# UoB-HPC/stdpar-nbody

Measured on AMD Instinct MI355X. Metric: body-steps/sec + %FP64 peak, 3D double all-pairs N=2^20 at 1/2/4/8 GPUs, higher is better.
Workload: dtype f64

## Files before the change

### stdpar-nbody_amd/csrc/all_pairs.hip

```cpp
#include "common.hpp"

#include <atomic>
#include <cstdlib>
#include <mutex>
#include <type_traits>
#include <vector>

namespace nbody {

constexpr int kBlock = 256;
constexpr int kWaves = kBlock / 64;

struct ap_config {
  int split = 0;
  int tpt   = 0;
  int path  = 0;
};
static std::atomic<uint32_t> g_ap_default{0};

static ap_config ap_config_of(const nbody_state* s) {
  const uint32_t t = s->tuning ? s->tuning : g_ap_default.load(std::memory_order_relaxed);
  ap_config c;
  c.split = int(t & 15u);
  c.tpt   = int((t >> 4) & 3u);
// ... 2 lines not shown
}

template <typename T, int D, int R, int JS>
__global__ __launch_bounds__(kBlock) void all_pairs_force_kernel(const T* __restrict__ m, const T* __restrict__ x,
                                                                 T* __restrict__ a, T c, uint32_t sz, uint32_t first,
                                                                 uint32_t count, const k1_rule* __restrict__ rule) {
  [[maybe_unused]] constexpr T e2 = T(0);
#define K1_SOFT false
#include "k1_tile_body.inc"
#undef K1_SOFT
}
template <typename T, int D, int R, int JS>
__global__ __launch_bounds__(kBlock) void all_pairs_softened_kernel(const T* __restrict__ m, const T* __restrict__ x,
                                                                    T* __restrict__ a, T c, uint32_t sz, uint32_t first,
                                                                    uint32_t count, T e2) {
  const k1_rule* const rule = nullptr;
#define K1_SOFT true
#include "k1_tile_body.inc"
#undef K1_SOFT
}

template <typename T, int D>
__global__ __launch_bounds__(kBlock) void pack_sources_kernel(const T* __restrict__ m, const T* __restrict__ x,
                                                              src_rec<T, D>* __restrict__ out, uint32_t sz, uint32_t padded) {
  const uint32_t j = blockIdx.x * kBlock + threadIdx.x;
  if (j >= padded) return;
  src_rec<T, D> r;
#pragma unroll
  for (int k = 0; k < 3; ++k) r.p[k] = (k < D && j < sz) ? x[uint64_t(j) * D + (k < D ? k : 0)] : T(0);
  r.m    = j < sz ? m[j] : T(0);
  out[j] = r;
}

template <typename T, int D, bool PACK, bool MOMENTS>
__global__ __launch_bounds__(kBlock) void k1_prepare_kernel(const T* __restrict__ m, const T* __restrict__ x, src_rec<T, D>* __restrict__ out,
                                                            cst_batch* __restrict__ cst, uint32_t sz, uint32_t padded, k1_rule* rule, double* partial,
                                                            uint32_t* turn, uint32_t turn_words) {
  const uint32_t j = blockIdx.x * kBlock + threadIdx.x;
  T p[D];
#pragma unroll
  for (int k = 0; k < D; ++k) p[k] = j < sz ? x[uint64_t(j) * D + k] : T(0);
  if constexpr (PACK) {
    if (j < padded) {
      src_rec<T, D> r;
#pragma unroll
      for (int k = 0; k < 3; ++k) r.p[k] = k < D ? p[k < D ? k : 0] : T(0);
      r.m    = j < sz ? m[j] : T(0);
      out[j] = r;
      if constexpr (sizeof(T) == 8) {
        const src_cst<T> k  = src_cst<T>::of(r.m);
        cst[j / 2].m15[j % 2]   = k.m15;
        cst[j / 2].m1875[j % 2] = k.m1875;
      }
    }
  }
  __shared__ double red[2 * D][kWaves];
  __shared__ bool last_s;
  const int lane = threadIdx.x & 63, wave = threadIdx.x >> 6;
  if constexpr (MOMENTS) {
    double s1[D], s2[D];
#pragma unroll
    for (int k = 0; k < D; ++k) {
      const double d = j < sz ? double(p[k]) - double(x[k]) : 0.0;
      s1[k] = d;
      s2[k] = d * d;
    }
#pragma unroll
    for (int k = 0; k < D; ++k)
      for (int off = 32; off > 0; off >>= 1) {
        s1[k] += __shfl_xor(s1[k], off, 64);
        s2[k] += __shfl_xor(s2[k], off, 64);
      }
    if (lane == 0) {
#pragma unroll
      for (int k = 0; k < D; ++k) {
        red[k][wave]     = s1[k];
        red[D + k][wave] = s2[k];
      }
    }
    __syncthreads();
    if (threadIdx.x < 2 * D) {
      double v = red[threadIdx.x][0];
      for (int w = 1; w < kWaves; ++w) v += red[threadIdx.x][w];
      __hip_atomic_store(partial + size_t(blockIdx.x) * (2 * D) + threadIdx.x, v, __ATOMIC_RELAXED, __HIP_MEMORY_SCOPE_AGENT);
    }
  }
  __builtin_amdgcn_s_waitcnt(0);
  __syncthreads();
  if (threadIdx.x == 0) last_s = __hip_atomic_fetch_add(&rule->ticket, 1u, __ATOMIC_RELAXED, __HIP_MEMORY_SCOPE_AGENT) == gridDim.x - 1u;
  __syncthreads();
  if (!last_s) return;
  if constexpr (MOMENTS) {
    double acc = 0.0;
    constexpr int G = kBlock / (2 * D), U = 8;
    const int q = threadIdx.x % (2 * D), g = threadIdx.x / (2 * D);
    if (g < G) {
      for (uint32_t b0 = uint32_t(g); b0 < gridDim.x; b0 += G * U) {
        double v[U];
#pragma unroll
        for (int u = 0; u < U; ++u) {
          const uint32_t b = b0 + uint32_t(u) * G;
          v[u] = b < gridDim.x ? __hip_atomic_load(partial + size_t(b) * (2 * D) + q, __ATOMIC_RELAXED, __HIP_MEMORY_SCOPE_AGENT) : 0.0;
        }
#pragma unroll
        for (int u = 0; u < U; ++u) acc += v[u];
      }
    }
    __shared__ double fin[kBlock];
    fin[threadIdx.x] = g < G ? acc : 0.0;
    __syncthreads();
    if (threadIdx.x < 2 * D) {
      double tot = 0.0;
#pragma unroll 6
      for (int gg = 0; gg < G; ++gg) tot += fin[gg * (2 * D) + threadIdx.x];
      fin[threadIdx.x] = tot;
    }
    __syncthreads();
    if (threadIdx.x == 0) {
      double vol = 1.0;
#pragma unroll
      for (int k = 0; k < D; ++k) {
        const double mean = fin[k] / double(sz), var = fin[D + k] / double(sz) - mean * mean;
        vol *= var > 0.0 ? __builtin_sqrt(12.0 * var) : 0.0;
      }
      rule->volume = vol;
      rule->sparse = vol >= kFarMinVolume<D> ? 1u : 0u;
    }
  }
  for (uint32_t w = threadIdx.x; w < turn_words; w += kBlock) turn[w] = 0u;
  if (threadIdx.x == 0) __hip_atomic_store(&rule->ticket, 0u, __ATOMIC_RELAXED, __HIP_MEMORY_SCOPE_AGENT);
}

template <int JS>
constexpr int kSgprWaves = JS > kWaves ? JS : kWaves;

constexpr uint32_t kTurnSpins  = 1u << 26;
constexpr uint32_t kTurnPoison = 0xffffffffu;
struct k1_status {
  uint32_t err, block, group, chunk;
  unsigned long long polls, waits;
};
struct k1_handoff {
  void* sums;
  uint32_t* turn;
  k1_status* status;
  uint32_t spins;
  uint32_t delay;
  uint32_t late;
};
template <typename T, int D, int R, int JS, int RULE = 0>
__global__ __launch_bounds__(64 * kSgprWaves<JS>) void all_pairs_force_sgpr_kernel(const src_rec<T, D>* __restrict__ packed,
                                                                                   const cst_batch* __restrict__ cst,
                                                                                   const T* __restrict__ x, T* a, T c, uint32_t sz,
                                                                                   uint32_t first, uint32_t count,
                                                                                   uint32_t tiles_per_chunk, k1_handoff h,
                                                                                   const k1_rule* __restrict__ rule) {
  [[maybe_unused]] constexpr T e2 = T(0);
#define K1_SOFT false
#include "k1_sgpr_body.inc"
#undef K1_SOFT
}
template <typename T, int D, int R, int JS>
__global__ __launch_bounds__(64 * kSgprWaves<JS>) void all_pairs_softened_sgpr_kernel(const src_rec<T, D>* __restrict__ packed,
                                                                                      const cst_batch* __restrict__ cst,
                                                                                      const T* __restrict__ x, T* a, T c, uint32_t sz,
                                                                                      uint32_t first, uint32_t count,
                                                                                      uint32_t tiles_per_chunk, k1_handoff h, T e2) {
  constexpr int RULE = 0;
  const k1_rule* const rule = nullptr;
#define K1_SOFT true
#include "k1_sgpr_body.inc"
#undef K1_SOFT
}

namespace {
struct scratch_buf {
  void* ptr  = nullptr;
  size_t cap = 0;
};
struct packed_slot {
  int device;
  hipStream_t stream;
  scratch_buf buf[7];
  std::vector<void*> retired;
  bool k1_dirty  = false;
  bool k1_failed = false;
};
std::mutex g_packed_mu;
std::vector<packed_slot> g_packed_slots;
}

int ap_scratch_get(hipStream_t st, int which, size_t bytes, void** out) {
  const int dev = stream_device(st);
  std::lock_guard<std::mutex> lock(g_packed_mu);
  packed_slot* slot = nullptr;
  for (auto& sl : g_packed_slots)
    if (sl.stream == st && sl.device == dev) slot = &sl;
  if (slot && slot->buf[which].cap >= bytes) {
    *out = slot->buf[which].ptr;
    return NBODY_OK;
  }
  hipStreamCaptureStatus cs = hipStreamCaptureStatusNone;
  if (st != nullptr) (void)hipStreamIsCapturing(st, &cs);
  if (cs != hipStreamCaptureStatusNone) {
    set_error("all-pairs: the scratch buffers of this stream must exist before a step is recorded "
              "(call nbody_all_pairs_force once outside nbody_graph_begin/end, or use a context from nbody_create)");
    return NBODY_ERR_STATE;
  }
  if (!slot) {
    g_packed_slots.push_back({dev, st, {}, {}});
    slot = &g_packed_slots.back();
  }
  void* fresh = nullptr;
  NB_HIP(hipMalloc(&fresh, bytes));
  if (which == 4 || which == 3) {
    if (hipError_t e = hipMemsetAsync(fresh, 0, bytes, st); e != hipSuccess) {
      (void)hipFree(fresh);
      return hip_fail(e, "hipMemsetAsync(K1 scratch)", __FILE__, __LINE__);
    }
  }
  if (slot->buf[which].ptr) slot->retired.push_back(slot->buf[which].ptr);
  slot->buf[which].ptr = fresh;
  slot->buf[which].cap = bytes;
  *out                 = fresh;
  return NBODY_OK;
}

void ap_scratch_release(hipStream_t st) {
  const int dev = stream_device(st);
  std::lock_guard<std::mutex> lock(g_packed_mu);
  for (size_t i = 0; i < g_packed_slots.size(); ++i) {
    if (g_packed_slots[i].stream == st && g_packed_slots[i].device == dev) {
      for (auto& b : g_packed_slots[i].buf) (void)hipFree(b.ptr);
      for (void* p : g_packed_slots[i].retired) (void)hipFree(p);
      g_packed_slots.erase(g_packed_slots.begin() + long(i));
      return;
    }
  }
}

struct k1_plan {
  bool scalar = false;
  int r = 1, js = 4;
  uint32_t chunks = 1, tiles_per_chunk = 0;
};

static int auto_split(uint32_t sz) { return sz >= 2048u ? 8 : 4; }

// ... 33 lines not shown
  if (p.r == 0) {
    const uint64_t blocks_r2 = (uint64_t(s->count) + 127) / 128 * p.chunks;
    if (p.scalar) p.r = (sizeof(T) == 8 && blocks_r2 >= 4096) ? 2 : 1;
    else p.r = blocks_r2 * uint64_t(p.js) >= 8192 ? 2 : 1;
  }
  *out = p;
  return NBODY_OK;
}

int ap_pack_sources(const nbody_state* s, hipStream_t st, void** packed_out) {
  const uint32_t padded = (s->sz + kTileJ - 1) / kTileJ * kTileJ;
  const size_t tsz      = s->dtype == NBODY_F32 ? 4 : 8;
  void* scratch         = nullptr;
  if (int r = ap_scratch_get(st, 0, 4 * tsz * size_t(padded), &scratch)) return r;
  int rc = dispatch(s->dtype, s->dim, [&](auto tg) {
    using T         = typename decltype(tg)::type;
    constexpr int D = decltype(tg)::dim;
    hipLaunchKernelGGL((pack_sources_kernel<T, D>), dim3((padded + kBlock - 1) / kBlock), dim3(kBlock), 0, st,
                       static_cast<const T*>(s->m), static_cast<const T*>(s->x), static_cast<src_rec<T, D>*>(scratch), s->sz, padded);
    NB_HIP(hipGetLastError());
    return int(NBODY_OK);
  });
  *packed_out = scratch;
  return rc;
}

static size_t ap_cst_bytes(size_t padded) { return sizeof(cst_batch) * (padded / 2); }

static size_t ap_rule_bytes(uint32_t sz, int dim) {
  const size_t padded = (size_t(sz) + kTileJ - 1) / kTileJ * kTileJ;
  return 32 + sizeof(double) * 2 * size_t(dim) * (padded / kBlock);
}

template <typename T, int D>
static int ap_prepare(const nbody_state* s, hipStream_t st, bool pack, src_rec<T, D>** packed_out, const cst_batch** cst_out,
                      const k1_rule** rule_out, uint32_t* turn, size_t turn_words, bool with_rule = true) {
  const uint32_t padded = (s->sz + kTileJ - 1) / kTileJ * kTileJ;
  const bool moments    = with_rule && s->sz >= kFarMinBodies;
  void* scratch         = nullptr;
  void* consts          = nullptr;
  if (pack) {
    if (int r = ap_scratch_get(st, 0, 4 * sizeof(T) * size_t(padded), &scratch)) return r;
    if (sizeof(T) == 8)
      if (int r = ap_scratch_get(st, 6, ap_cst_bytes(padded), &consts)) return r;
  }
  void* q = nullptr;
  if (int r = ap_scratch_get(st, 3, ap_rule_bytes(s->sz, D), &q)) return r;
  auto* rule    = static_cast<k1_rule*>(q);
  auto* partial = reinterpret_cast<double*>(static_cast<char*>(q) + 32);
  auto* out     = static_cast<src_rec<T, D>*>(scratch);
  auto* cst     = static_cast<cst_batch*>(consts);
  const dim3 grid(padded / kBlock), block(kBlock);
  const T *m = static_cast<const T*>(s->m), *x = static_cast<const T*>(s->x);
  const uint32_t words = uint32_t(turn_words);
  if (pack && moments) hipLaunchKernelGGL((k1_prepare_kernel<T, D, true, true>), grid, block, 0, st, m, x, out, cst, s->sz, padded, rule, partial, turn, words);
  else if (pack) hipLaunchKernelGGL((k1_prepare_kernel<T, D, true, false>), grid, block, 0, st, m, x, out, cst, s->sz, padded, rule, partial, turn, words);
  else if (moments) hipLaunchKernelGGL((k1_prepare_kernel<T, D, false, true>), grid, block, 0, st, m, x, out, cst, s->sz, padded, rule, partial, turn, words);
  NB_HIP(hipGetLastError());
  if (packed_out) *packed_out = out;
  if (cst_out) *cst_out = cst;
  *rule_out = moments ? rule : nullptr;
  return NBODY_OK;
}

constexpr uint32_t kCollectMaxBlocks = 2048;
static bool k1_collect(uint32_t target_blocks, uint32_t chunks) {
  uint32_t limit = kCollectMaxBlocks;
  if (const char* e = experiment_env("NBODY_K1_COLLECT_MAX")) limit = uint32_t(atoi(e));
  return chunks > 1 && uint64_t(target_blocks) * chunks <= limit;
}
template <typename T, int D, int R, int JS>
static size_t k1_collect_bytes(uint32_t target_blocks, uint32_t chunks) {
  constexpr int TG = kSgprWaves<JS> / JS;
  return sizeof(T) * size_t(chunks) * target_blocks * TG * R * D * 64;
}

template <int R, int JS>
static size_t sgpr_turn_words(uint32_t count) {
  constexpr int TG = kSgprWaves<JS> / JS, TB = TG * 64 * R;
  return size_t((count + TB - 1) / TB) * TG;
}

template <typename T, int D, int R, int JS, bool SOFT>
static int launch_all_pairs_sgpr(const nbody_state* s, const k1_plan& plan, hipStream_t st, T e2) {
  constexpr int TB = (kSgprWaves<JS> / JS) * 64 * R;
  uint32_t blocks  = (s->count + TB - 1) / TB;
  if (blocks == 0) return NBODY_OK;
  k1_handoff h{nullptr, nullptr, nullptr, kTurnSpins, 0u, 0u};
  if (plan.chunks > 1) {
    void* q = nullptr;
    if (int r = ap_scratch_get(st, 1, sizeof(uint32_t) * sgpr_turn_words<R, JS>(s->count), &q)) return r;
    h.turn = static_cast<uint32_t*>(q);
    if (k1_collect(blocks, plan.chunks)) {
      if (int r = ap_scratch_get(st, 5, k1_collect_bytes<T, D, R, JS>(blocks, plan.chunks), &q)) return r;
      h.sums = q;
    }
    if (int r = ap_scratch_get(st, 4, sizeof(k1_status), &q)) return r;
    h.status = static_cast<k1_status*>(q);
    if (const char* e = experiment_env("NBODY_K1_TURN_SPINS")) h.spins = uint32_t(strtoul(e, nullptr, 10));
    if (const char* e = experiment_env("NBODY_K1_HANDOFF_DELAY")) h.delay = uint32_t(strtoul(e, nullptr, 10));
    if (const char* e = experiment_env("NBODY_K1_HANDOFF_LATE")) h.late = uint32_t(strtoul(e, nullptr, 10));
    if (const char* e = experiment_env("NBODY_K1_NO_HANDOFF"); e && e[0] == '1') h.turn = nullptr, h.sums = nullptr;
    if (const char* e = experiment_env("NBODY_K1_COLLECT"); e && e[0] == '0') h.sums = nullptr;
  }
  src_rec<T, D>* packed = nullptr;
  const cst_batch* cst  = nullptr;
  const k1_rule* rule   = nullptr;
  if (int r = ap_prepare<T, D>(s, st, true, &packed, &cst, &rule, h.turn, h.turn ? sgpr_turn_words<R, JS>(s->count) : 0, !SOFT)) return r;
  if constexpr (SOFT) {
    hipLaunchKernelGGL((all_pairs_softened_sgpr_kernel<T, D, R, JS>), dim3(blocks, plan.chunks), dim3(64 * kSgprWaves<JS>), 0, st,
                       packed, cst, static_cast<const T*>(s->x), static_cast<T*>(s->a), static_cast<T>(s->c), s->sz, s->first, s->count,
                       plan.tiles_per_chunk, h, e2);
    NB_HIP(hipGetLastError());
    if (h.turn != nullptr && h.sums == nullptr) ap_status_mark(st);
    return NBODY_OK;
  }
#ifdef NBODY_EXPERIMENTS
  if (const char* e = getenv("NBODY_K1_RULE_FORCE"); e && JS == 8 && D == 3) {
    if (e[0] == '1')
      hipLaunchKernelGGL((all_pairs_force_sgpr_kernel<T, D, R, JS, 1>), dim3(blocks, plan.chunks), dim3(64 * kSgprWaves<JS>), 0, st,
                         packed, cst, static_cast<const T*>(s->x), static_cast<T*>(s->a), static_cast<T>(s->c), s->sz, s->first, s->count,
                         plan.tiles_per_chunk, h, rule);
    else
      hipLaunchKernelGGL((all_pairs_force_sgpr_kernel<T, D, R, JS, 2>), dim3(blocks, plan.chunks), dim3(64 * kSgprWaves<JS>), 0, st,
                         packed, cst, static_cast<const T*>(s->x), static_cast<T*>(s->a), static_cast<T>(s->c), s->sz, s->first, s->count,
                         plan.tiles_per_chunk, h, rule);
    NB_HIP(hipGetLastError());
    return NBODY_OK;
  }
#endif
  hipLaunchKernelGGL((all_pairs_force_sgpr_kernel<T, D, R, JS>), dim3(blocks, plan.chunks), dim3(64 * kSgprWaves<JS>), 0, st,
                     packed, cst, static_cast<const T*>(s->x), static_cast<T*>(s->a), static_cast<T>(s->c), s->sz, s->first, s->count,
                     plan.tiles_per_chunk, h, rule);
  NB_HIP(hipGetLastError());
  if (h.turn != nullptr && h.sums == nullptr) ap_status_mark(st);
  return NBODY_OK;
}

template <typename T, int D, int R, int JS, bool SOFT>
static int launch_all_pairs(const nbody_state* s, hipStream_t st, T e2) {
  constexpr int TB = (kWaves / JS) * 64 * R;
  uint32_t blocks  = (s->count + TB - 1) / TB;
  if (blocks == 0) return NBODY_OK;
  if constexpr (SOFT) {
    hipLaunchKernelGGL((all_pairs_softened_kernel<T, D, R, JS>), dim3(blocks), dim3(kBlock), 0, st, static_cast<const T*>(s->m),
                       static_cast<const T*>(s->x), static_cast<T*>(s->a), static_cast<T>(s->c), s->sz, s->first, s->count, e2);
    NB_HIP(hipGetLastError());
    return NBODY_OK;
  }
  const k1_rule* rule = nullptr;
  if (int r = ap_prepare<T, D>(s, st, false, nullptr, nullptr, &rule, nullptr, 0)) return r;
  hipLaunchKernelGGL((all_pairs_force_kernel<T, D, R, JS>), dim3(blocks), dim3(kBlock), 0, st, static_cast<const T*>(s->m),
                     static_cast<const T*>(s->x), static_cast<T*>(s->a), static_cast<T>(s->c), s->sz, s->first, s->count, rule);
  NB_HIP(hipGetLastError());
  return NBODY_OK;
}

template <typename F>
static bool with_k1_instance(const k1_plan& p, F&& fn) {
#define NB_CASE(RR, JJ)                                                                       \
  if (p.r == RR && p.js == JJ) {                                                              \
    fn(std::integral_constant<int, RR>{}, std::integral_constant<int, JJ>{});                 \
    return true;                                                                              \
  }
  NB_CASE(1, 1);
  NB_CASE(1, 2);
// ... 9 lines not shown
  return false;
}

template <typename T, int D, bool SOFT = false>
static int all_pairs_dispatch(const nbody_state* s, hipStream_t st, T e2 = T(0)) {
  k1_plan p;
  if (int rc = plan_all_pairs<T>(s, &p)) return rc;
  int rc = NBODY_OK;
  const bool found = with_k1_instance(p, [&](auto r, auto js) {
    constexpr int R = decltype(r)::value, JS = decltype(js)::value;
    rc = p.scalar ? launch_all_pairs_sgpr<T, D, R, JS, SOFT>(s, p, st, e2)
                  : (JS <= kWaves ? launch_all_pairs<T, D, R, (JS <= kWaves ? JS : 1), SOFT>(s, st, e2) : int(NBODY_ERR_ARG));
  });
  if (!found) {
    set_error("all-pairs: unsupported config split=%d targets_per_thread=%d", p.js, p.r);
    return NBODY_ERR_ARG;
  }
  return rc;
}

template <typename T, int D>
static int all_pairs_describe(const nbody_state* s, char* out, size_t len) {
  k1_plan p;
  if (int rc = plan_all_pairs<T>(s, &p)) return rc;
  const char* t = sizeof(T) == 8 ? "double" : "float";
  const char* pair = sizeof(T) == 4 ? (s->sz >= kFarMinBodies ? "rsq+rcp[m y^3 at r2 >= 4 if sparse]" : "rsq+rcp")
                                    : s->sz >= kFarMinBodies ? "far3m[-eps if sparse]/near3" : "far3m/near3";
  if (p.scalar) {
    bool collect = false;
    with_k1_instance(p, [&](auto r, auto js) {
      constexpr int TB = (kSgprWaves<decltype(js)::value> / decltype(js)::value) * 64 * decltype(r)::value;
      collect = k1_collect((s->count + TB - 1) / TB, p.chunks);
    });
    snprintf(out, len, "all_pairs_force_sgpr_kernel<%s,%d,R=%d,JS=%d> tile=%d chunks=%u%s pair=%s", t, D, p.r, p.js, kTileJ, p.chunks,
             p.chunks > 1 ? (collect ? "(summed in chunk order by the last to arrive)" : "(summed in turn into a)") : "", pair);
  }
  else
    snprintf(out, len, "all_pairs_force_kernel<%s,%d,R=%d,JS=%d> tile=%d chunks=1 pair=%s", t, D, p.r, p.js, kTileJ, pair);
  return NBODY_OK;
}

int ap_scratch_reserve(hipStream_t st, const nbody_state* s) {
  void* q             = nullptr;
  const size_t tsz    = s->dtype == NBODY_F32 ? 4 : 8;
  const size_t padded = (size_t(s->sz) + 2 * kTileJ - 1) / (2 * kTileJ) * (2 * kTileJ);
  if (int r = ap_scratch_get(st, 0, 4 * tsz * padded, &q)) return r;
  if (s->dtype == NBODY_F64)
    if (int r = ap_scratch_get(st, 6, ap_cst_bytes(padded), &q)) return r;
  if (int r = ap_scratch_get(st, 3, ap_rule_bytes(s->sz, s->dim), &q)) return r;
  return dispatch(s->dtype, s->dim, [&](auto tg) {
    using T = typename decltype(tg)::type;
    k1_plan p;
    if (int rc = plan_all_pairs<T>(s, &p)) return rc;
    if (!p.scalar || p.chunks <= 1) return int(NBODY_OK);
    size_t words = 0;
    with_k1_instance(p, [&](auto r, auto js) { words = sgpr_turn_words<decltype(r)::value, decltype(js)::value>(s->count); });
    if (!words) return int(NBODY_OK);
    if (int rc = ap_scratch_get(st, 1, sizeof(uint32_t) * words, &q)) return rc;
    size_t sums = 0;
    with_k1_instance(p, [&](auto r, auto js) {
      constexpr int RR = decltype(r)::value, JJ = decltype(js)::value;
      const uint32_t blocks = (s->count + (kSgprWaves<JJ> / JJ) * 64 * RR - 1) / ((kSgprWaves<JJ> / JJ) * 64 * RR);
      if (k1_collect(blocks, p.chunks)) sums = k1_collect_bytes<T, decltype(tg)::dim, RR, JJ>(blocks, p.chunks);
    });
    if (sums)
      if (int rc = ap_scratch_get(st, 5, sums, &q)) return rc;
    return ap_scratch_get(st, 4, sizeof(k1_status), &q);
  });
}

void ap_status_mark(hipStream_t st) {
  const int dev = stream_device(st);
  std::lock_guard<std::mutex> lock(g_packed_mu);
  for (auto& sl : g_packed_slots)
    if (sl.stream == st && sl.device == dev) sl.k1_dirty = true;
}

int ap_status_read(hipStream_t st, unsigned long long out[6], bool clear) {
  const int dev = stream_device(st);
  k1_status* dptr = nullptr;
  {
    std::lock_guard<std::mutex> lock(g_packed_mu);
// ... 610 lines not shown
  });
}

extern "C" int nbody_all_pairs_force(const nbody_state* s, void* stream) {
  if (int r = check_state(s)) return r;
  device_guard guard(stream_device(as_stream(stream)));
  return dispatch(s->dtype, s->dim, [&](auto tg) {
    using TG = decltype(tg);
    return all_pairs_dispatch<typename TG::type, TG::dim>(s, as_stream(stream));
  });
}

extern "C" int nbody_all_pairs_softened_force(const nbody_state* s, double eps, void* stream) {
  if (int r = check_state(s)) return r;
  return dispatch(s->dtype, s->dim, [&](auto tg) {
    using TG = decltype(tg);
    using T  = typename TG::type;
    T e2;
    if (int r = check_softening<T>(eps, &e2)) return r;
    device_guard guard(stream_device(as_stream(stream)));
    return all_pairs_dispatch<T, TG::dim, true>(s, as_stream(stream), e2);
  });
}

extern "C" int nbody_all_pairs_status(void* stream, uint64_t out[6], int clear) {
  device_guard guard(stream_device(as_stream(stream)));
  unsigned long long v[6] = {0, 0, 0, 0, 0, 0};
  const int rc = ap_status_read(as_stream(stream), v, clear != 0);
  if (out)
    for (int i = 0; i < 6; ++i) out[i] = v[i];
  return rc;
}

extern "C" int nbody_all_pairs_collapsed_force(const nbody_state* s, void* stream) {
  if (int r = check_state(s)) return r;
  device_guard guard(stream_device(as_stream(stream)));
  return dispatch(s->dtype, s->dim, [&](auto tg) {
    using TG = decltype(tg);
    return collapsed_dispatch<typename TG::type, TG::dim>(s, as_stream(stream));
  });
}

extern "C" int nbody_accelerate_step(const nbody_state* s, void* stream) {
  if (int r = check_state(s)) return r;
  device_guard guard(stream_device(as_stream(stream)));
  return dispatch(s->dtype, s->dim, [&](auto tg) {
    using TG = decltype(tg);
    return accelerate_dispatch<typename TG::type, TG::dim>(s, as_stream(stream));
  });
}
```

### stdpar-nbody_amd/csrc/common.hpp

```cpp
#pragma once
#include <hip/hip_runtime.h>

#include <cfloat>
#include <cstdarg>
#include <cstdint>
#include <cstdio>
#include <cstdlib>
#include <cstring>

#include "../../include/nbody_hip.h"

namespace nbody {

void set_error(const char* fmt, ...);
int hip_fail(hipError_t e, const char* what, const char* file, int line);

#define NB_HIP(call)                                                                   \
  do {                                                                                 \
    hipError_t e_ = (call);                                                            \
    if (e_ != hipSuccess) return ::nbody::hip_fail(e_, #call, __FILE__, __LINE__);     \
  } while (0)

#define NB_ARG(cond, ...)                \
  do {                                   \
// ... 343 lines not shown
#pragma unroll
      for (int u = 0; u < U; ++u)
#pragma unroll
        for (int r = 0; r < R; ++r) w[u][r] = pair_math<T>::template weight_far_folded<false>(r2[u][r], s[u].m, kc[u].m15, kc[u].m1875);
    } else {
#pragma unroll
      for (int u = 0; u < U; ++u)
#pragma unroll
        for (int r = 0; r < R; ++r) {
          const uint32_t hi = uint32_t(__builtin_bit_cast(unsigned long long, r2[u][r]) >> 32);
          const T mine      = hi < pair_math<T>::far_hi ? pc.keps : T(0);
          w[u][r]           = pair_math<T>::template weight_far_folded<true>(r2[u][r], s[u].m, kc[u].m15, kc[u].m1875, mine);
        }
      if (__builtin_expect(__builtin_amdgcn_ballot_w64(lowest < pair_math<T>::near_hi) != 0ull, 0)) {
#pragma unroll
        for (int u = 0; u < U; ++u)
#pragma unroll
          for (int r = 0; r < R; ++r) {
            const uint32_t hi = uint32_t(__builtin_bit_cast(unsigned long long, r2[u][r]) >> 32);
            const T wn        = pair_math<T>::template weight<3>(r2[u][r], s[u].m);
            w[u][r]           = hi < pair_math<T>::near_hi ? wn : w[u][r];
          }
      }
    }
#pragma unroll
    for (int u = 0; u < U; ++u)
#pragma unroll
      for (int r = 0; r < R; ++r)
#pragma unroll
        for (int k = 0; k < D; ++k) acc[r][k] = __builtin_elementwise_fma(w[u][r], d[u][r][k], acc[r][k]);
  }
}

template <typename T, int D, int R, int U, bool ffar>
__device__ __forceinline__ void pair_batch(T (&acc)[R][D], const T (&xi)[R][D], const src_rec<T, D> (&s)[U], const pair_consts<T>& pc) {
  static_assert(sizeof(T) == 4, "f64 callers pass the sources' constants (src_cst)");
  const src_cst<T> none[U] = {};
  pair_batch<T, D, R, U, ffar>(acc, xi, s, none, pc);
}

template <typename T>
__device__ __forceinline__ T soft_weight(T q, T mj, const pair_consts<T>& pc) {
  if constexpr (sizeof(T) == 8) {
    return pair_math<double>::template weight_far<false>(q, mj, pc.k15, pc.k1875);
  } else {
    const T y = __builtin_amdgcn_rsqf(q);
    return mj * ((y * y) * y);
  }
}

template <typename T, int D, int R, int U, bool SSRC = false>
__device__ __forceinline__ void pair_batch_soft(T (&acc)[R][D], const T (&xi)[R][D], const src_rec<T, D> (&s)[U],
                                                const src_cst<T> (&kc)[U], const pair_consts<T>& pc, T e2) {
  T d[U][R][D], q[U][R], w[U][R];
#pragma unroll
  for (int u = 0; u < U; ++u)
#pragma unroll
    for (int r = 0; r < R; ++r) {
#pragma unroll
      for (int k = 0; k < D; ++k) d[u][r][k] = s[u].p[k] - xi[r][k];
      T t = e2;
#pragma unroll
      for (int k = 0; k < D; ++k) t = __builtin_elementwise_fma(d[u][r][k], d[u][r][k], t);
      q[u][r] = t;
    }
#pragma unroll
// ... 12 lines not shown
      for (int k = 0; k < D; ++k) acc[r][k] = __builtin_elementwise_fma(w[u][r], d[u][r][k], acc[r][k]);
}

template <typename T>
constexpr T kSoftMinE2 = sizeof(T) == 4 ? T(0x1p-84f) : T(0x1p-680);

template <typename T>
inline int check_softening(double eps, T* e2_out) {
  NB_ARG(eps > 0.0 && eps <= DBL_MAX, "softening length eps = %g must be finite and > 0", eps);
  const T te = T(eps);
  const T e2 = te * te;
  NB_ARG(e2 >= kSoftMinE2<T> && e2 <= (sizeof(T) == 4 ? T(FLT_MAX) : T(DBL_MAX)),
         "softening length eps = %g: eps^2 = %g in %s is outside [%g, max]: its square must be a normal number whose ^(-3/2) is finite",
         eps, double(e2), sizeof(T) == 4 ? "float" : "double", double(kSoftMinE2<T>));
  *e2_out = e2;
  return NBODY_OK;
}

inline hipStream_t as_stream(void* s) { return reinterpret_cast<hipStream_t>(s); }

struct k1_rule {
  double volume;
  uint32_t sparse;
  uint32_t ticket;
};
constexpr uint32_t kFarMinBodies = 32768;
template <int D>
constexpr double kFarMinVolume = D == 3 ? 1.7e5 : 6.4e4;
__device__ __forceinline__ bool ap_far_mode(const k1_rule* __restrict__ rule) {
  if (rule == nullptr) return false;
  return __builtin_amdgcn_readfirstlane(int(rule->sparse)) != 0;
}

constexpr int kTileJ = 512;

typedef uint32_t sgpr16 __attribute__((ext_vector_type(16)));
template <typename V>
__device__ __forceinline__ sgpr16 sload16(const void* p, V& tie) {
  sgpr16 r;
  asm volatile("s_load_dwordx16 %0, %2, 0x0" : "=s"(r), "+v"(tie) : "s"(p));
  return r;
}
template <typename V>
__device__ __forceinline__ void swait(sgpr16& v, V& tie) {
  asm volatile("s_waitcnt lgkmcnt(0)" : "+s"(v), "+v"(tie));
}

typedef uint32_t reg4 __attribute__((ext_vector_type(4)));
struct cst_regs {
  reg4 v, s;
};
template <typename V>
__device__ __forceinline__ cst_regs cload(const void* p, uint32_t vzero, V& tie) {
  cst_regs r;
  asm volatile("global_load_dwordx4 %0, %3, %4\n\ts_load_dwordx4 %1, %4, 0x10" : "=&v"(r.v), "=&s"(r.s), "+v"(tie) : "v"(vzero), "s"(p));
  return r;
}
template <typename V>
__device__ __forceinline__ void cswait(sgpr16& v, cst_regs& c, V& tie) {
  asm volatile("s_waitcnt vmcnt(0) lgkmcnt(0)" : "+s"(v), "+v"(c.v), "+s"(c.s), "+v"(tie));
}
__device__ __forceinline__ void cst_unpack(const cst_regs& c, src_cst<double> (&kc)[2]) {
  struct pair_t {
    double d[2];
  };
  const pair_t v = __builtin_bit_cast(pair_t, c.v), s = __builtin_bit_cast(pair_t, c.s);
// ... 22 lines not shown
```

### stdpar-nbody_amd/csrc/k1_sgpr_body.inc

```
  using rec_t = src_rec<T, D>;
  constexpr int TG  = kSgprWaves<JS> / JS;
  constexpr int TB  = TG * 64 * R;
  constexpr int SUB = kTileJ / JS;
  __shared__ T partial[(JS > 1) ? (JS - 1) * TG * 64 * R * D : 1];
  const int lane   = threadIdx.x & 63;
  const int wave   = __builtin_amdgcn_readfirstlane(threadIdx.x >> 6);
  const int tgroup = wave / JS;
  const int jpart  = wave % JS;
  T xi[R][D], acc[R][D];
  uint32_t ti[R];
#pragma unroll
  for (int r = 0; r < R; ++r) {
    uint32_t local = blockIdx.x * TB + tgroup * (64 * R) + r * 64 + lane;
    ti[r]          = local;
    uint64_t i     = uint64_t(first) + (local < count ? local : 0u);
#pragma unroll
    for (int k = 0; k < D; ++k) {
      xi[r][k]  = x[i * D + k];
      acc[r][k] = T(0);
    }
  }
  const uint32_t ntiles = (sz + kTileJ - 1) / kTileJ;
  const uint32_t t0     = blockIdx.y * tiles_per_chunk;
  const uint32_t t1     = min(ntiles, t0 + tiles_per_chunk);
  const pair_consts<T> pc;
  const bool ffar       = !K1_SOFT && ap_far_mode(rule);
  const uint32_t nsteps = (t1 - t0) * SUB;
  constexpr int U = 64 / int(sizeof(rec_t));
  struct batch_t {
    rec_t r[U];
  };
  auto batch = [&](uint32_t k) { return packed + (uint64_t(t0 + k / SUB) * kTileJ + uint32_t(jpart) * SUB + (k % SUB)); };
  constexpr bool CST = sizeof(T) == 8;
  auto cbatch = [&](uint32_t k) { return cst + (uint64_t(t0 + k / SUB) * kTileJ + uint32_t(jpart) * SUB + (k % SUB)) / U; };
  [[maybe_unused]] uint32_t vzero = 0;
  if constexpr (CST) {
    asm volatile("" : "+v"(vzero));
#pragma unroll
    for (int r = 0; r < R; ++r)
#pragma unroll
      for (int k = 0; k < D; ++k) asm volatile("" : "+v"(xi[r][k]));
  }
  auto run = [&](auto ff) {
    constexpr bool FF = decltype(ff)::value;
    sgpr16 A, B;
    [[maybe_unused]] cst_regs CA, CB;
    auto request = [&](sgpr16& S, cst_regs& C, uint32_t k) {
      if constexpr (CST) C = cload(cbatch(k), vzero, xi[0][0]);
      S = sload16(batch(k), xi[0][0]);
    };
    auto wait = [&](sgpr16& S, cst_regs& C) {
      if constexpr (CST) cswait(S, C, acc[0][0]);
      else swait(S, acc[0][0]);
    };
    auto consume = [&](const sgpr16& S, const cst_regs& C) {
      const batch_t b = __builtin_bit_cast(batch_t, S);
      src_cst<T> kc[U];
      if constexpr (CST) cst_unpack(C, kc);
      if constexpr (K1_SOFT) pair_batch_soft<T, D, R, U, true>(acc, xi, b.r, kc, pc, e2);
      else pair_batch<T, D, R, U, FF>(acc, xi, b.r, kc, pc);
    };
    request(A, CA, 0);
    for (uint32_t k = 0; k < nsteps; k += 2 * U) {
      wait(A, CA);
      request(B, CB, k + U);
      consume(A, CA);
      wait(B, CB);
      request(A, CA, k + 2 * U < nsteps ? k + 2 * U : k);
      consume(B, CB);
    }
    wait(A, CA);
  };
  if constexpr (K1_SOFT) run(std::false_type{});
  else if constexpr (RULE == 1) run(std::false_type{});
  else if constexpr (RULE == 2) run(std::true_type{});
  else if (ffar) run(std::true_type{});
  else run(std::false_type{});
  if constexpr (JS > 1) {
    if (jpart > 0) {
#pragma unroll
      for (int r = 0; r < R; ++r)
#pragma unroll
        for (int k = 0; k < D; ++k) partial[((((jpart - 1) * TG + tgroup) * R + r) * D + k) * 64 + lane] = acc[r][k];
    }
    __syncthreads();
    if (jpart == 0) {
#pragma unroll
      for (int p = 1; p < JS; ++p)
#pragma unroll
        for (int r = 0; r < R; ++r)
#pragma unroll
          for (int k = 0; k < D; ++k) acc[r][k] += partial[((((p - 1) * TG + tgroup) * R + r) * D + k) * 64 + lane];
    }
  }
  if (jpart != 0) return;
  const uint32_t y = blockIdx.y, last = gridDim.y - 1u;
  uint32_t* const tw = h.turn + blockIdx.x * TG + tgroup;
  if (h.sums != nullptr) {
    const size_t group_scalars = size_t(R) * D * 64;
    T* const all  = static_cast<T*>(h.sums);
    T* const mine = all + ((size_t(y) * gridDim.x + blockIdx.x) * TG + tgroup) * group_scalars;
#pragma unroll
    for (int r = 0; r < R; ++r)
#pragma unroll
      for (int k = 0; k < D; ++k) __hip_atomic_store(mine + (r * D + k) * 64 + lane, acc[r][k], __ATOMIC_RELAXED, __HIP_MEMORY_SCOPE_AGENT);
    __builtin_amdgcn_s_waitcnt(0);
    __builtin_amdgcn_wave_barrier();
    uint32_t drawn = 0;
    if (lane == 0) drawn = __hip_atomic_fetch_add(tw, 1u, __ATOMIC_RELAXED, __HIP_MEMORY_SCOPE_AGENT);
    if (uint32_t(__builtin_amdgcn_readfirstlane(int(drawn))) != last) return;
// ... 102 lines not shown
```

Measured before the change: 1.766 million.

## Certify far-field blocks via per-chunk bounding boxes to skip the r2 test

The prepare kernel now also reduces per-block and per-chunk bounding boxes of source positions. In the force kernel, each block checks whether all of its targets lie at least a fixed gap from the chunk's box. When they do, it runs a far-only pair routine that skips the per-pair near/far r2 branch. This adds reduction work and scratch memory in the prepare step, plus a code path whose correctness depends on the gap being large enough.

```diff
diff --git a/stdpar-nbody_amd/csrc/all_pairs.hip b/stdpar-nbody_amd/csrc/all_pairs.hip
--- a/stdpar-nbody_amd/csrc/all_pairs.hip
+++ b/stdpar-nbody_amd/csrc/all_pairs.hip
@@ -58,10 +58,26 @@
   out[j] = r;
 }
 
+template <typename T>
+struct k1_prepare_tail {
+  uint32_t turn_words;
+};
+template <>
+struct k1_prepare_tail<double> {
+  uint32_t turn_words;
+  uint32_t bpc;
+  double* cbox;
+  double* pbox;
+};
 template <typename T, int D, bool PACK, bool MOMENTS>
 __global__ __launch_bounds__(kBlock) void k1_prepare_kernel(const T* __restrict__ m, const T* __restrict__ x, src_rec<T, D>* __restrict__ out,
                                                             cst_batch* __restrict__ cst, uint32_t sz, uint32_t padded, k1_rule* rule, double* partial,
-                                                            uint32_t* turn, uint32_t turn_words) {
+                                                            uint32_t* turn, k1_prepare_tail<T> tail) {
+  constexpr bool BOX        = PACK && MOMENTS && sizeof(T) == 8;
+  const uint32_t turn_words = tail.turn_words;
+  [[maybe_unused]] uint32_t bpc = 0;
+  [[maybe_unused]] T *cbox = nullptr, *pbox = nullptr;
+  if constexpr (BOX) bpc = tail.bpc, cbox = tail.cbox, pbox = tail.pbox;
   const uint32_t j = blockIdx.x * kBlock + threadIdx.x;
   T p[D];
 #pragma unroll
@@ -81,6 +97,7 @@
     }
   }
   __shared__ double red[2 * D][kWaves];
+  __shared__ T bred[BOX ? 2 * D : 1][kWaves];
   __shared__ bool last_s;
   const int lane = threadIdx.x & 63, wave = threadIdx.x >> 6;
   if constexpr (MOMENTS) {
@@ -104,11 +121,45 @@
         red[D + k][wave] = s2[k];
       }
     }
+    if constexpr (BOX) {
+      if (bpc != 0) {
+        bool finite = true;
+#pragma unroll
+        for (int k = 0; k < D; ++k) finite = finite && (p[k] - p[k]) == T(0);
+        T lo[D], hi[D];
+#pragma unroll
+        for (int k = 0; k < D; ++k) {
+          lo[k] = finite ? p[k] : -T(__builtin_inf());
+          hi[k] = finite ? p[k] : T(__builtin_inf());
+        }
+#pragma unroll
+        for (int k = 0; k < D; ++k)
+          for (int off = 32; off > 0; off >>= 1) {
+            lo[k] = __builtin_fmin(lo[k], __shfl_xor(lo[k], off, 64));
+            hi[k] = __builtin_fmax(hi[k], __shfl_xor(hi[k], off, 64));
+          }
+        if (lane == 0) {
+#pragma unroll
+          for (int k = 0; k < D; ++k) {
+            bred[k][wave]     = lo[k];
+            bred[D + k][wave] = hi[k];
+          }
+        }
+      }
+    }
     __syncthreads();
     if (threadIdx.x < 2 * D) {
       double v = red[threadIdx.x][0];
       for (int w = 1; w < kWaves; ++w) v += red[threadIdx.x][w];
       __hip_atomic_store(partial + size_t(blockIdx.x) * (2 * D) + threadIdx.x, v, __ATOMIC_RELAXED, __HIP_MEMORY_SCOPE_AGENT);
+    }
+    if constexpr (BOX) {
+      if (bpc != 0 && threadIdx.x >= 64 && threadIdx.x < 64 + 2 * D) {
+        const int q = int(threadIdx.x) - 64;
+        T v         = bred[q][0];
+        for (int w = 1; w < kWaves; ++w) v = q < D ? __builtin_fmin(v, bred[q][w]) : __builtin_fmax(v, bred[q][w]);
+        __hip_atomic_store(pbox + size_t(blockIdx.x) * (2 * D) + q, v, __ATOMIC_RELAXED, __HIP_MEMORY_SCOPE_AGENT);
+      }
     }
   }
   __builtin_amdgcn_s_waitcnt(0);
@@ -151,6 +202,50 @@
       }
       rule->volume = vol;
       rule->sparse = vol >= kFarMinVolume<D> ? 1u : 0u;
+    }
+  }
+  if constexpr (BOX) {
+    if (bpc != 0) {
+      const uint32_t nchunks = (gridDim.x + bpc - 1) / bpc;
+      const uint32_t sub     = threadIdx.x & 15u;
+      for (uint32_t c0 = 0; c0 < nchunks; c0 += kBlock / 16) {
+        const uint32_t c  = c0 + (threadIdx.x >> 4);
+        const uint32_t b1 = c < nchunks ? min(gridDim.x, (c + 1u) * bpc) : 0u;
+        T lo[D], hi[D];
+#pragma unroll
+        for (int k = 0; k < D; ++k) lo[k] = T(__builtin_inf()), hi[k] = -T(__builtin_inf());
+        for (uint32_t b0 = c * bpc + sub; b0 < b1; b0 += 16u * 4u) {
+          T v[4][2 * D];
+#pragma unroll
+          for (int u = 0; u < 4; ++u) {
+            const uint32_t b = b0 + 16u * uint32_t(u);
+#pragma unroll
+            for (int q = 0; q < 2 * D; ++q)
+              v[u][q] = b < b1 ? __hip_atomic_load(pbox + size_t(b) * (2 * D) + q, __ATOMIC_RELAXED, __HIP_MEMORY_SCOPE_AGENT)
+                               : (q < D ? T(__builtin_inf()) : -T(__builtin_inf()));
+          }
+#pragma unroll
+          for (int u = 0; u < 4; ++u)
+#pragma unroll
+            for (int k = 0; k < D; ++k) {
+              lo[k] = __builtin_fmin(lo[k], v[u][k]);
+              hi[k] = __builtin_fmax(hi[k], v[u][D + k]);
+            }
+        }
+#pragma unroll
+        for (int k = 0; k < D; ++k)
+          for (int off = 8; off > 0; off >>= 1) {
+            lo[k] = __builtin_fmin(lo[k], __shfl_xor(lo[k], off, 64));
+            hi[k] = __builtin_fmax(hi[k], __shfl_xor(hi[k], off, 64));
+          }
+        if (c < nchunks && sub == 0) {
+#pragma unroll
+          for (int k = 0; k < D; ++k) {
+            cbox[size_t(c) * (2 * D) + k]     = lo[k];
+            cbox[size_t(c) * (2 * D) + D + k] = hi[k];
+          }
+        }
+      }
     }
   }
   for (uint32_t w = threadIdx.x; w < turn_words; w += kBlock) turn[w] = 0u;
@@ -174,14 +269,27 @@
   uint32_t delay;
   uint32_t late;
 };
+constexpr size_t kBoxHeaderBytes = 64;
+template <typename T>
+struct k1_rule_arg {
+  const k1_rule* rule;
+};
+template <>
+struct k1_rule_arg<double> {
+  const k1_rule* rule;
+  const double* box;
+};
 template <typename T, int D, int R, int JS, int RULE = 0>
 __global__ __launch_bounds__(64 * kSgprWaves<JS>) void all_pairs_force_sgpr_kernel(const src_rec<T, D>* __restrict__ packed,
                                                                                    const cst_batch* __restrict__ cst,
                                                                                    const T* __restrict__ x, T* a, T c, uint32_t sz,
                                                                                    uint32_t first, uint32_t count,
                                                                                    uint32_t tiles_per_chunk, k1_handoff h,
-                                                                                   const k1_rule* __restrict__ rule) {
+                                                                                   k1_rule_arg<T> ra) {
   [[maybe_unused]] constexpr T e2 = T(0);
+  const k1_rule* __restrict__ const rule = ra.rule;
+  [[maybe_unused]] const T* __restrict__ box = nullptr;
+  if constexpr (sizeof(T) == 8) box = ra.box;
 #define K1_SOFT false
 #include "k1_sgpr_body.inc"
 #undef K1_SOFT
@@ -194,6 +302,7 @@
                                                                                       uint32_t tiles_per_chunk, k1_handoff h, T e2) {
   constexpr int RULE = 0;
   const k1_rule* const rule = nullptr;
+  [[maybe_unused]] const T* const box = nullptr;
 #define K1_SOFT true
 #include "k1_sgpr_body.inc"
 #undef K1_SOFT
@@ -207,7 +316,7 @@
 struct packed_slot {
   int device;
   hipStream_t stream;
-  scratch_buf buf[7];
+  scratch_buf buf[8];
   std::vector<void*> retired;
   bool k1_dirty  = false;
   bool k1_failed = false;
@@ -239,7 +348,7 @@
   }
   void* fresh = nullptr;
   NB_HIP(hipMalloc(&fresh, bytes));
-  if (which == 4 || which == 3) {
+  if (which == 4 || which == 3 || which == 7) {
     if (hipError_t e = hipMemsetAsync(fresh, 0, bytes, st); e != hipSuccess) {
       (void)hipFree(fresh);
       return hip_fail(e, "hipMemsetAsync(K1 scratch)", __FILE__, __LINE__);
@@ -339,9 +448,16 @@
   return 32 + sizeof(double) * 2 * size_t(dim) * (padded / kBlock);
 }
 
+static size_t ap_box_bytes(uint32_t sz, int dim) {
+  const size_t ntiles = (size_t(sz) + kTileJ - 1) / kTileJ;
+  return kBoxHeaderBytes + sizeof(double) * 2 * size_t(dim) * (ntiles + ntiles * (kTileJ / kBlock));
+}
+static bool k1_box_wanted(uint32_t sz, uint32_t chunks) { return sz >= kFarMinBodies && chunks > 1; }
+
 template <typename T, int D>
 static int ap_prepare(const nbody_state* s, hipStream_t st, bool pack, src_rec<T, D>** packed_out, const cst_batch** cst_out,
-                      const k1_rule** rule_out, uint32_t* turn, size_t turn_words, bool with_rule = true) {
+                      const k1_rule** rule_out, uint32_t* turn, size_t turn_words, bool with_rule = true, uint32_t box_tpc = 0,
+                      const T** box_out = nullptr) {
   const uint32_t padded = (s->sz + kTileJ - 1) / kTileJ * kTileJ;
   const bool moments    = with_rule && s->sz >= kFarMinBodies;
   void* scratch         = nullptr;
@@ -357,13 +473,26 @@
   auto* partial = reinterpret_cast<double*>(static_cast<char*>(q) + 32);
   auto* out     = static_cast<src_rec<T, D>*>(scratch);
   auto* cst     = static_cast<cst_batch*>(consts);
+  T *cbox = nullptr, *pbox = nullptr;
+  uint32_t bpc = 0;
+  if (sizeof(T) == 8 && pack && moments && box_tpc != 0) {
+    void* b = nullptr;
+    if (int r = ap_scratch_get(st, 7, ap_box_bytes(s->sz, D), &b)) return r;
+    cbox = reinterpret_cast<T*>(static_cast<char*>(b) + kBoxHeaderBytes);
+    pbox = cbox + size_t(2 * D) * (padded / kTileJ);
+    bpc  = box_tpc * (kTileJ / kBlock);
+  }
   const dim3 grid(padded / kBlock), block(kBlock);
   const T *m = static_cast<const T*>(s->m), *x = static_cast<const T*>(s->x);
   const uint32_t words = uint32_t(turn_words);
-  if (pack && moments) hipLaunchKernelGGL((k1_prepare_kernel<T, D, true, true>), grid, block, 0, st, m, x, out, cst, s->sz, padded, rule, partial, turn, words);
-  else if (pack) hipLaunchKernelGGL((k1_prepare_kernel<T, D, true, false>), grid, block, 0, st, m, x, out, cst, s->sz, padded, rule, partial, turn, words);
-  else if (moments) hipLaunchKernelGGL((k1_prepare_kernel<T, D, false, true>), grid, block, 0, st, m, x, out, cst, s->sz, padded, rule, partial, turn, words);
+  k1_prepare_tail<T> tail{};
+  tail.turn_words = words;
+  if constexpr (sizeof(T) == 8) tail.bpc = bpc, tail.cbox = cbox, tail.pbox = pbox;
+  if (pack && moments) hipLaunchKernelGGL((k1_prepare_kernel<T, D, true, true>), grid, block, 0, st, m, x, out, cst, s->sz, padded, rule, partial, turn, tail);
+  else if (pack) hipLaunchKernelGGL((k1_prepare_kernel<T, D, true, false>), grid, block, 0, st, m, x, out, cst, s->sz, padded, rule, partial, turn, tail);
+  else if (moments) hipLaunchKernelGGL((k1_prepare_kernel<T, D, false, true>), grid, block, 0, st, m, x, out, cst, s->sz, padded, rule, partial, turn, tail);
   NB_HIP(hipGetLastError());
+  if (box_out) *box_out = cbox;
   if (packed_out) *packed_out = out;
   if (cst_out) *cst_out = cst;
   *rule_out = moments ? rule : nullptr;
@@ -413,7 +542,12 @@
   src_rec<T, D>* packed = nullptr;
   const cst_batch* cst  = nullptr;
   const k1_rule* rule   = nullptr;
-  if (int r = ap_prepare<T, D>(s, st, true, &packed, &cst, &rule, h.turn, h.turn ? sgpr_turn_words<R, JS>(s->count) : 0, !SOFT)) return r;
+  const T* box          = nullptr;
+  bool certify          = !SOFT && sizeof(T) == 8 && k1_box_wanted(s->sz, plan.chunks);
+  if (const char* e = experiment_env("NBODY_K1_NO_CERT"); e && e[0] == '1') certify = false;
+  if (int r = ap_prepare<T, D>(s, st, true, &packed, &cst, &rule, h.turn, h.turn ? sgpr_turn_words<R, JS>(s->count) : 0, !SOFT,
+                               certify ? plan.tiles_per_chunk : 0u, &box))
+    return r;
   if constexpr (SOFT) {
     hipLaunchKernelGGL((all_pairs_softened_sgpr_kernel<T, D, R, JS>), dim3(blocks, plan.chunks), dim3(64 * kSgprWaves<JS>), 0, st,
                        packed, cst, static_cast<const T*>(s->x), static_cast<T*>(s->a), static_cast<T>(s->c), s->sz, s->first, s->count,
@@ -422,23 +556,26 @@
     if (h.turn != nullptr && h.sums == nullptr) ap_status_mark(st);
     return NBODY_OK;
   }
+  k1_rule_arg<T> ra{};
+  ra.rule = rule;
+  if constexpr (sizeof(T) == 8) ra.box = box;
 #ifdef NBODY_EXPERIMENTS
   if (const char* e = getenv("NBODY_K1_RULE_FORCE"); e && JS == 8 && D == 3) {
     if (e[0] == '1')
       hipLaunchKernelGGL((all_pairs_force_sgpr_kernel<T, D, R, JS, 1>), dim3(blocks, plan.chunks), dim3(64 * kSgprWaves<JS>), 0, st,
                          packed, cst, static_cast<const T*>(s->x), static_cast<T*>(s->a), static_cast<T>(s->c), s->sz, s->first, s->count,
-                         plan.tiles_per_chunk, h, rule);
+                         plan.tiles_per_chunk, h, ra);
     else
       hipLaunchKernelGGL((all_pairs_force_sgpr_kernel<T, D, R, JS, 2>), dim3(blocks, plan.chunks), dim3(64 * kSgprWaves<JS>), 0, st,
                          packed, cst, static_cast<const T*>(s->x), static_cast<T*>(s->a), static_cast<T>(s->c), s->sz, s->first, s->count,
-                         plan.tiles_per_chunk, h, rule);
+                         plan.tiles_per_chunk, h, ra);
     NB_HIP(hipGetLastError());
     return NBODY_OK;
   }
 #endif
   hipLaunchKernelGGL((all_pairs_force_sgpr_kernel<T, D, R, JS>), dim3(blocks, plan.chunks), dim3(64 * kSgprWaves<JS>), 0, st,
                      packed, cst, static_cast<const T*>(s->x), static_cast<T*>(s->a), static_cast<T>(s->c), s->sz, s->first, s->count,
-                     plan.tiles_per_chunk, h, rule);
+                     plan.tiles_per_chunk, h, ra);
   NB_HIP(hipGetLastError());
   if (h.turn != nullptr && h.sums == nullptr) ap_status_mark(st);
   return NBODY_OK;
@@ -514,8 +651,9 @@
       constexpr int TB = (kSgprWaves<decltype(js)::value> / decltype(js)::value) * 64 * decltype(r)::value;
       collect = k1_collect((s->count + TB - 1) / TB, p.chunks);
     });
-    snprintf(out, len, "all_pairs_force_sgpr_kernel<%s,%d,R=%d,JS=%d> tile=%d chunks=%u%s pair=%s", t, D, p.r, p.js, kTileJ, p.chunks,
-             p.chunks > 1 ? (collect ? "(summed in chunk order by the last to arrive)" : "(summed in turn into a)") : "", pair);
+    snprintf(out, len, "all_pairs_force_sgpr_kernel<%s,%d,R=%d,JS=%d> tile=%d chunks=%u%s pair=%s%s", t, D, p.r, p.js, kTileJ, p.chunks,
+             p.chunks > 1 ? (collect ? "(summed in chunk order by the last to arrive)" : "(summed in turn into a)") : "", pair,
+             sizeof(T) == 8 && k1_box_wanted(s->sz, p.chunks) ? " cert=box-gap>=3[if sparse: blocks proven far skip the r2 test]" : "");
   }
   else
     snprintf(out, len, "all_pairs_force_kernel<%s,%d,R=%d,JS=%d> tile=%d chunks=1 pair=%s", t, D, p.r, p.js, kTileJ, pair);
@@ -530,6 +668,8 @@
   if (s->dtype == NBODY_F64)
     if (int r = ap_scratch_get(st, 6, ap_cst_bytes(padded), &q)) return r;
   if (int r = ap_scratch_get(st, 3, ap_rule_bytes(s->sz, s->dim), &q)) return r;
+  if (s->dtype == NBODY_F64 && s->sz >= kFarMinBodies)
+    if (int r = ap_scratch_get(st, 7, ap_box_bytes(s->sz, s->dim), &q)) return r;
   return dispatch(s->dtype, s->dim, [&](auto tg) {
     using T = typename decltype(tg)::type;
     k1_plan p;
@@ -1206,6 +1346,30 @@
   return rc;
 }
 
+#ifdef NBODY_EXPERIMENTS
+extern "C" int nbody_exp_k1_certified(void* stream, uint64_t* out, int clear) {
+  NB_ARG(out != nullptr, "out is NULL");
+  hipStream_t st = as_stream(stream);
+  const int dev  = stream_device(st);
+  device_guard guard(dev);
+  void* dptr = nullptr;
+  {
+    std::lock_guard<std::mutex> lock(g_packed_mu);
+    for (auto& sl : g_packed_slots)
+      if (sl.stream == st && sl.device == dev) dptr = sl.buf[7].ptr;
+  }
+  unsigned long long v = 0;
+  if (dptr) NB_HIP(hipMemcpyAsync(&v, dptr, sizeof v, hipMemcpyDeviceToHost, st));
+  NB_HIP(hipStreamSynchronize(st));
+  if (dptr && clear) {
+    NB_HIP(hipMemsetAsync(dptr, 0, sizeof v, st));
+    NB_HIP(hipStreamSynchronize(st));
+  }
+  *out = v;
+  return NBODY_OK;
+}
+#endif
+
 extern "C" int nbody_all_pairs_collapsed_force(const nbody_state* s, void* stream) {
   if (int r = check_state(s)) return r;
   device_guard guard(stream_device(as_stream(stream)));
diff --git a/stdpar-nbody_amd/csrc/common.hpp b/stdpar-nbody_amd/csrc/common.hpp
--- a/stdpar-nbody_amd/csrc/common.hpp
+++ b/stdpar-nbody_amd/csrc/common.hpp
@@ -399,6 +399,34 @@
   }
 }
 
+template <typename T, int D, int R, int U>
+__device__ __forceinline__ void pair_batch_far(T (&acc)[R][D], const T (&xi)[R][D], const src_rec<T, D> (&s)[U], const src_cst<T> (&kc)[U]) {
+  static_assert(sizeof(T) == 8, "the certified copy exists in f64 only");
+  T d[U][R][D], r2[U][R], w[U][R];
+#pragma unroll
+  for (int u = 0; u < U; ++u)
+#pragma unroll
+    for (int r = 0; r < R; ++r) {
+#pragma unroll
+      for (int k = 0; k < D; ++k) d[u][r][k] = s[u].p[k] - xi[r][k];
+      T q = pair_math<T>::tiny;
+#pragma unroll
+      for (int k = 0; k < D; ++k) q = __builtin_elementwise_fma(d[u][r][k], d[u][r][k], q);
+      r2[u][r] = q;
+    }
+#pragma unroll
+  for (int u = 0; u < U; ++u)
+#pragma unroll
+    for (int r = 0; r < R; ++r)
+      w[u][r] = pair_math<T>::template weight_far_folded<false, R == 1>(r2[u][r], s[u].m, kc[u].m15, kc[u].m1875);
+#pragma unroll
+  for (int u = 0; u < U; ++u)
+#pragma unroll
+    for (int r = 0; r < R; ++r)
+#pragma unroll
+      for (int k = 0; k < D; ++k) acc[r][k] = __builtin_elementwise_fma(w[u][r], d[u][r][k], acc[r][k]);
+}
+
 template <typename T, int D, int R, int U, bool ffar>
 __device__ __forceinline__ void pair_batch(T (&acc)[R][D], const T (&xi)[R][D], const src_rec<T, D> (&s)[U], const pair_consts<T>& pc) {
   static_assert(sizeof(T) == 4, "f64 callers pass the sources' constants (src_cst)");
@@ -477,6 +505,29 @@
   return __builtin_amdgcn_readfirstlane(int(rule->sparse)) != 0;
 }
 
+constexpr double kFarGap = 3.0;
+template <typename T, int D, int R>
+__device__ __forceinline__ bool k1_block_is_far(const T (&xi)[R][D], const T __attribute__((address_space(4))) * chunk_box) {
+  bool far = false, finite = true;
+#pragma unroll
+  for (int r = 0; r < R; ++r)
+#pragma unroll
+    for (int k = 0; k < D; ++k) finite = finite & ((xi[r][k] - xi[r][k]) == T(0));
+#pragma unroll
+  for (int k = 0; k < D; ++k) {
+    const T lo = chunk_box[k], hi = chunk_box[D + k];
+    bool above = true, below = true;
+#pragma unroll
+    for (int r = 0; r < R; ++r) {
+      const T ga = xi[r][k] - hi, gb = lo - xi[r][k];
+      above = above & (ga >= T(kFarGap));
+      below = below & (gb >= T(kFarGap));
+    }
+    far = far | (__builtin_amdgcn_ballot_w64(!above) == 0ull) | (__builtin_amdgcn_ballot_w64(!below) == 0ull);
+  }
+  return far & (__builtin_amdgcn_ballot_w64(!finite) == 0ull);
+}
+
 constexpr int kTileJ = 512;
 
 typedef uint32_t sgpr16 __attribute__((ext_vector_type(16)));
diff --git a/stdpar-nbody_amd/csrc/k1_sgpr_body.inc b/stdpar-nbody_amd/csrc/k1_sgpr_body.inc
--- a/stdpar-nbody_amd/csrc/k1_sgpr_body.inc
+++ b/stdpar-nbody_amd/csrc/k1_sgpr_body.inc
@@ -41,8 +41,18 @@
 #pragma unroll
       for (int k = 0; k < D; ++k) asm volatile("" : "+v"(xi[r][k]));
   }
+  [[maybe_unused]] bool cfar = false;
+  if constexpr (!K1_SOFT && CST && RULE == 0) {
+    if (ffar && box != nullptr) {
+      cfar = k1_block_is_far<T, D, R>(xi, (const T __attribute__((address_space(4)))*)(box + size_t(blockIdx.y) * (2 * D)));
+#ifdef NBODY_EXPERIMENTS
+      if (cfar && jpart == 0 && lane == 0)
+        atomicAdd(reinterpret_cast<unsigned long long*>(const_cast<T*>(box)) - kBoxHeaderBytes / 8, 1ull);
+#endif
+    }
+  }
   auto run = [&](auto ff) {
-    constexpr bool FF = decltype(ff)::value;
+    constexpr int FF = int(decltype(ff)::value);
     sgpr16 A, B;
     [[maybe_unused]] cst_regs CA, CB;
     auto request = [&](sgpr16& S, cst_regs& C, uint32_t k) {
@@ -58,7 +68,8 @@
       src_cst<T> kc[U];
       if constexpr (CST) cst_unpack(C, kc);
       if constexpr (K1_SOFT) pair_batch_soft<T, D, R, U, true>(acc, xi, b.r, kc, pc, e2);
-      else pair_batch<T, D, R, U, FF>(acc, xi, b.r, kc, pc);
+      else if constexpr (FF == 2) pair_batch_far<T, D, R, U>(acc, xi, b.r, kc);
+      else pair_batch<T, D, R, U, FF != 0>(acc, xi, b.r, kc, pc);
     };
     request(A, CA, 0);
     for (uint32_t k = 0; k < nsteps; k += 2 * U) {
@@ -74,8 +85,12 @@
   if constexpr (K1_SOFT) run(std::false_type{});
   else if constexpr (RULE == 1) run(std::false_type{});
   else if constexpr (RULE == 2) run(std::true_type{});
-  else if (ffar) run(std::true_type{});
-  else run(std::false_type{});
+  else if (ffar) {
+    if constexpr (CST) {
+      if (cfar) run(std::integral_constant<int, 2>{});
+      else run(std::true_type{});
+    } else run(std::true_type{});
+  } else run(std::false_type{});
   if constexpr (JS > 1) {
     if (jpart > 0) {
 #pragma unroll
```

After: 1.804 million, median of 6. +2.2%, better.
